# deryrahman/image-caption-emotion-indonesia

Hardware: AMD Instinct MI355X
Metric: images/sec (train step) + NLL loss match, batch=64 ResNet152+FactoredLSTM-512 (higher is better)
Workload: dtype f32 (trunk: operands as 2 f16 pieces each, 3 MFMA products per multiply, f32 accumulate; decoder: large products as 3 bf16 pieces per operand, 6 MFMA products per multiply, the rest f32 MFMA; the persistent LSTM kernel the trunk's split-f16 scheme)

## Files before the change

### image-caption-emotion-indonesia_amd/csrc/fused_block.hip

```cpp
#include <cstdlib>
#include <type_traits>

#include "common.h"
#include "mfma_core.h"
#include "split_f16.h"
#include "kernels.h"

namespace capnet {
namespace {

__host__ __device__ constexpr int fb_kslot(int g, int j) { return 16 * (j >> 2) + 4 * g + (j & 3); }


__global__ __launch_bounds__(256) void fb_pack_kernel(const float* __restrict__ w, unsigned* __restrict__ img, int C, int MID,
                                                      int role, int wide) {
  const int ew = f16x3_weight_shift(img[1]);
  if (blockIdx.x == 0 && threadIdx.x == 0) { img[0] = (unsigned)ew; img[2] = (unsigned)wide; }
  const float ws = ldexpf(1.f, ew);
  const long cells = (long)C * MID / 8 * 2;
  for (long i = (long)blockIdx.x * blockDim.x + threadIdx.x; i < cells; i += (long)gridDim.x * blockDim.x) {
    long r = i;
    const int lane = (int)(r & 63); r >>= 6;
    const int plane = (int)(r & 1); r >>= 1;
    const float* src;
// ... 109 lines not shown
      }
#pragma unroll
      for (int c = 0; c < 4; ++c) {
        const f32x4 a = {x[0][c], x[1][c], x[2][c], x[3][c]}, b = {x[4][c], x[5][c], x[6][c], x[7][c]};
        h4 ha, la, hb, lb;
        split4(a, ha, la);
        split4(b, hb, lb);
        unsigned char* d = lds + (rg * K + 4 * chq + c) * 16;
        *reinterpret_cast<h8*>(d) = cat8(ha, hb);
        *reinterpret_cast<h8*>(d + kPlane) = cat8(la, lb);
      }
    }
  };
  auto mma = [&]() __attribute__((always_inline)) {
#pragma unroll 2
    for (int k = 0; k < NRG / 2; ++k) {
      const unsigned char* base = lds + ((2 * k + lh) * K + li) * 16;
      h8 ah[NBLK], al[NBLK], bh[NBLK], bl[NBLK];
#pragma unroll
      for (int b = 0; b < NBLK; ++b) {
        ah[b] = *reinterpret_cast<const h8*>(base + (b * 64 + wm * 32) * 16);
        al[b] = *reinterpret_cast<const h8*>(base + (b * 64 + wm * 32) * 16 + kPlane);
        bh[b] = *reinterpret_cast<const h8*>(base + (b * 64 + wn * 32) * 16);
        bl[b] = *reinterpret_cast<const h8*>(base + (b * 64 + wn * 32) * 16 + kPlane);
      }
      int p = 0;
#pragma unroll
      for (int bi = 0; bi < NBLK; ++bi)
#pragma unroll
        for (int bj = bi; bj < NBLK; ++bj, ++p) {
          acc[p] = __builtin_amdgcn_mfma_f32_32x32x16_f16(al[bi], bh[bj], acc[p], 0, 0, 0);
          acc[p] = __builtin_amdgcn_mfma_f32_32x32x16_f16(ah[bi], bl[bj], acc[p], 0, 0, 0);
          acc[p] = __builtin_amdgcn_mfma_f32_32x32x16_f16(ah[bi], bh[bj], acc[p], 0, 0, 0);
        }
    }
  };
  fetch(0);
  for (int st = 0; st < nst; ++st) {
    stage(st);
    __syncthreads();
    fetch(st + 1 < nst ? st + 1 : st);
    mma();
    __syncthreads();
  }
  const float osc = ldexpf(1.f, -2 * g.in_exp);
#pragma unroll
  for (int p = 0; p < NPAIR; ++p) {
#pragma unroll
    for (int r = 0; r < 16; ++r) {
      const int m = wm * 32 + (r & 3) + 8 * (r >> 2) + 4 * lh;
      g.gp[(((long)p * 64 + m) * g.slices + slice) * 64 + wn * 32 + li] = acc[p][r] * osc;
    }
  }
  f32x4* cs_sh = reinterpret_cast<f32x4*>(lds);
  cs_sh[tid] = colsum;
  __syncthreads();
  if (tid < NCQ) {
    f32x4 t = cs_sh[tid];
#pragma unroll
    for (int q = 1; q < 256 / NCQ; ++q) t += cs_sh[q * NCQ + tid];
    *reinterpret_cast<f32x4*>(g.cs + (long)slice * K + 4 * tid) = t * ldexpf(1.f, -g.in_exp);
  }
}

__global__ __launch_bounds__(256) void fb_gram_reduce_kernel(const float* __restrict__ gp, const float* __restrict__ cs, float* __restrict__ G,
                                                             float* __restrict__ mu, int K, int slices, int pairs) {
  __shared__ double sh[8][32][4];
  const int it = threadIdx.x & 31, part = threadIdx.x >> 5;
  const int item_wgs = pairs * 32;
  if ((int)blockIdx.x < item_wgs) {
    const int item = blockIdx.x * 32 + it;
    const int n4 = item & 15, m = (item >> 4) & 63, pair = item >> 10;
    const float* p = gp + ((long)(pair * 64 + m) * slices) * 64 + 4 * n4;
    double s[4] = {0.0, 0.0, 0.0, 0.0};
    for (int s0 = part; s0 < slices; s0 += 64) {
      f32x4 v[8];
#pragma unroll
      for (int u = 0; u < 8; ++u) {
        const int sl = s0 + 8 * u;
        v[u] = *reinterpret_cast<const f32x4*>(p + (long)(sl < slices ? sl : part) * 64);
      }
#pragma unroll
      for (int u = 0; u < 8; ++u)
#pragma unroll
        for (int i = 0; i < 4; ++i) s[i] += (s0 + 8 * u < slices) ? (double)v[u][i] : 0.0;
    }
#pragma unroll
    for (int i = 0; i < 4; ++i) sh[part][it][i] = s[i];
    __syncthreads();
    if (part == 0) {
#pragma unroll
      for (int q = 1; q < 8; ++q)
#pragma unroll
        for (int i = 0; i < 4; ++i) s[i] += sh[q][it][i];
      const int nb = K / 64;
      int bi = 0, bj = pair;
      while (bj >= nb - bi) { bj -= nb - bi; ++bi; }
      bj += bi;
      const int r = bi * 64 + m, c = bj * 64 + 4 * n4;
      const f32x4 o = {(float)s[0], (float)s[1], (float)s[2], (float)s[3]};
      *reinterpret_cast<f32x4*>(G + (long)r * K + c) = o;
      if (bi < bj) {
#pragma unroll
        for (int i = 0; i < 4; ++i) G[(long)(c + i) * K + r] = o[i];
      }
    }
  } else {
    const int e = ((int)blockIdx.x - item_wgs) * 32 + it;
    double s = 0.0;
    if (e < K) {
      const float* p = cs + e;
      for (int s0 = part; s0 < slices; s0 += 64) {
        float v[8];
#pragma unroll
        for (int u = 0; u < 8; ++u) {
          const int sl = s0 + 8 * u;
          v[u] = p[(long)(sl < slices ? sl : part) * K];
        }
#pragma unroll
        for (int u = 0; u < 8; ++u) s += (s0 + 8 * u < slices) ? (double)v[u] : 0.0;
      }
    }
    sh[part][it][0] = s;
    __syncthreads();
    if (part == 0 && e < K) {
#pragma unroll
      for (int q = 1; q < 8; ++q) s += sh[q][it][0];
      mu[e] = (float)s;
    }
  }
}

constexpr int kQC = 16;

template <int K>
__global__ __launch_bounds__(K * 4) void fb_quad_kernel(const float* __restrict__ G, const float* __restrict__ mu,
                                                        const float* __restrict__ w , int C, double inv_count,
                                                        double unbias, const float* __restrict__ gamma, const float* __restrict__ beta,
                                                        float* __restrict__ running_mean, float* __restrict__ running_var,
                                                        float momentum, float eps, float* __restrict__ scale, float* __restrict__ shift,
                                                        float* __restrict__ batch_mean, float* __restrict__ batch_var, int* __restrict__ err) {
  constexpr int NW = K / 16, S = K / 4, SB = S < 32 ? S : 32;
  __shared__ float red[2][kQC][NW];
  const int tid = threadIdx.x, lane = tid & 63, nb = tid >> 6, g4 = lane >> 4, ln = lane & 15, c0 = blockIdx.x * kQC;
  const float* wq = w + (long)blockIdx.x * K * kQC;
  f32x4 acc = {0.f, 0.f, 0.f, 0.f};
#pragma unroll
  for (int s0 = 0; s0 < S; s0 += SB) {
    float a[SB], b[SB];
#pragma unroll
    for (int i = 0; i < SB; ++i) {
      const int k = 4 * (s0 + i) + g4;
      a[i] = wq[k * kQC + ln];
      b[i] = G[(long)k * K + 16 * nb + ln];
    }
#pragma unroll
    for (int i = 0; i < SB; ++i) acc = __builtin_amdgcn_mfma_f32_16x16x4f32(a[i], b[i], acc, 0, 0, 0);
  }
  const int col = 16 * nb + ln;
  const f32x4 wv = *reinterpret_cast<const f32x4*>(wq + col * kQC + 4 * g4);
  const float m = mu[col];
#pragma unroll
  for (int r = 0; r < 4; ++r) {
    float q = acc[r] * wv[r], sm = m * wv[r];
#pragma unroll
    for (int o = 1; o < 16; o <<= 1) {
      q += __shfl_xor(q, o);
      sm += __shfl_xor(sm, o);
    }
    if (ln == 0) { red[0][4 * g4 + r][nb] = q; red[1][4 * g4 + r][nb] = sm; }
  }
  __syncthreads();
  if (tid < kQC && c0 + tid < C) {
    const int c = c0 + tid;
    double qq = 0.0, ss = 0.0;
#pragma unroll
    for (int v = 0; v < NW; ++v) { qq += (double)red[0][tid][v]; ss += (double)red[1][tid][v]; }
    if (err && !(qq < __builtin_inf())) atomicOr(err, 8);
    const double mean = ss * inv_count;
    double var = qq * inv_count - mean * mean;
    if (var < 0.0) var = 0.0;
    const float invstd = (float)(1.0 / sqrt(var + (double)eps));
    const float gm = gamma ? gamma[c] : 1.f, bt = beta ? beta[c] : 0.f;
    const float sc = gm * invstd;
    scale[c] = sc;
    shift[c] = bt - (float)mean * sc;
    if (running_mean) {
      running_mean[c] = __builtin_fmaf(momentum, (float)mean, (1.f - momentum) * running_mean[c]);
      running_var[c] = __builtin_fmaf(momentum, (float)(var * unbias), (1.f - momentum) * running_var[c]);
    }
    if (batch_mean) {
      batch_mean[c] = (float)mean;
      batch_var[c] = (float)(var * unbias);
    }
  }
}

struct FArgs {
  const float* y2; const float* s2; const float* t2;
  const unsigned* w3; const unsigned* w1;
  const float* s3; const float* t3;
  const float* res; const float* sd; const float* td;
  float* out; float* y1; float* part_sum; float* part_sq;
  int M, e3, e1;
  int* err;
};

#ifndef CAPNET_FB_DBG
#define CAPNET_FB_DBG 0
#endif

template <int MID, int RS, int NW>
__global__ __launch_bounds__(64 * NW, NW / 4) void fb_fused_kernel(const FArgs g) {
  constexpr int C = 4 * MID, KS = MID / 32, NB = MID / 16, NCH = C / 32;
  constexpr int SLOT = MID * 128;
  constexpr int NDMA = SLOT / 1024 / NW;
  constexpr int L = 2 * RS;
  constexpr int TR = 16 * RS * NW;
  constexpr int NT = 64 * NW;
  static_assert(NDMA >= 1 && 4 * NDMA + 2 * L <= 63, "vmcnt range");
  __shared__ __attribute__((aligned(16))) unsigned char ring[4 * SLOT];
  __shared__ __attribute__((aligned(16))) float par[4][C];
  const int tid = threadIdx.x, lane = tid & 63, wave = tid >> 6, gq = lane >> 4, ln = lane & 15;
  const int wave_u = __builtin_amdgcn_readfirstlane(wave);
  const unsigned ring0 = __builtin_amdgcn_readfirstlane((unsigned)(size_t)(__attribute__((address_space(3))) unsigned char*)ring);
  const int tile0 = (int)blockIdx.x * TR;
  const bool fold_res = g.sd != nullptr;
  const float* const w3img = reinterpret_cast<const float*>(g.w3 + kF16x3HdrWords);
  const float* const w1img = reinterpret_cast<const float*>(g.w1 + kF16x3HdrWords);

  auto dma = [&](const float* img, int cc, int slot) __attribute__((always_inline)) {
    const float* src = img + (long)cc * (SLOT / 4);
#pragma unroll
    for (int q = 0; q < ((CAPNET_FB_DBG == 2 || CAPNET_FB_DBG == 4) ? 0 : NDMA); ++q)
      glds16(src, (wave_u * NDMA + q) * 1024 + lane * 16, ring0 + (unsigned)(slot * SLOT + (wave_u * NDMA + q) * 1024));
  };
  unsigned idoff[RS];
#pragma unroll
  for (int s = 0; s < RS; ++s) {
    const int row = min(tile0 + (wave * RS + s) * 16 + ln, g.M - 1);
    idoff[s] = (unsigned)(((long)row * C + 4 * gq) * 4);
  }
  f32x4 idA[RS][2], idB[RS][2];
  auto fetch_id = [&](int cc, f32x4 (&id)[RS][2]) __attribute__((always_inline)) {
#pragma unroll
    for (int s = 0; s < RS; ++s)
#pragma unroll
      for (int blk = 0; blk < 2; ++blk) gload16(id[s][blk], g.res, idoff[s] + (unsigned)((32 * cc + 16 * blk) * 4));
  };

  dma(w3img, 0, 0);
  dma(w1img, 0, 1);
  fetch_id(0, idA);
  fetch_id(NCH > 1 ? 1 : 0, idB);
  {
    const float x3 = f16x3_out_scale(g.w3[0], g.e3);
    for (int i = tid; i < C; i += NT) {
      par[0][i] = g.s3[i] * x3;
      par[1][i] = g.t3[i];
      par[2][i] = fold_res ? g.sd[i] : 1.f;
      par[3][i] = fold_res ? g.td[i] : 0.f;
    }
  }
  h8 ah[RS][KS], al[RS][KS];
  {
    const float is3 = ldexpf(1.f, g.e3);
#pragma unroll
    for (int s = 0; s < RS; ++s) {
      const int row = min(tile0 + (wave * RS + s) * 16 + ln, g.M - 1);
      const float* p = g.y2 + (long)row * MID + 4 * gq;
#pragma unroll
      for (int ks = 0; ks < KS; ++ks) {
        f32x4 v0 = *reinterpret_cast<const f32x4*>(p + 32 * ks), v1 = *reinterpret_cast<const f32x4*>(p + 32 * ks + 16);
        const f32x4 sa = *reinterpret_cast<const f32x4*>(g.s2 + 32 * ks + 4 * gq), sb = *reinterpret_cast<const f32x4*>(g.s2 + 32 * ks + 16 + 4 * gq);
        const f32x4 ta = *reinterpret_cast<const f32x4*>(g.t2 + 32 * ks + 4 * gq), tb = *reinterpret_cast<const f32x4*>(g.t2 + 32 * ks + 16 + 4 * gq);
#pragma unroll
        for (int e = 0; e < 4; ++e) {
          v0[e] = fmaxf(fmaf(v0[e], sa[e], ta[e]), 0.f) * is3;
          v1[e] = fmaxf(fmaf(v1[e], sb[e], tb[e]), 0.f) * is3;
        }
        h4 h0, l0, h1, l1;
        split4(v0, h0, l0);
        split4(v1, h1, l1);
        ah[s][ks] = cat8(h0, h1);
        al[s][ks] = cat8(l0, l1);
      }
    }
  }
  wait_vmcnt<0>();
  CAPNET_LANDED4(idA[0][0], idA[0][1], idB[0][0], idB[0][1]);
  if constexpr (RS == 2) CAPNET_LANDED4(idA[1][0], idA[1][1], idB[1][0], idB[1][1]);
  __syncthreads();

  f32x4 acc[RS][NB];
#pragma unroll
  for (int s = 0; s < RS; ++s)
#pragma unroll
    for (int nb = 0; nb < NB; ++nb) acc[s][nb] = f32x4{0.f, 0.f, 0.f, 0.f};
  const float is1 = ldexpf(1.f, g.e1);

#ifndef CAPNET_FB_GB8
#define CAPNET_FB_GB8 2
#endif
  constexpr int GB = NW == 8 ? CAPNET_FB_GB8 : 4;
#ifndef CAPNET_FB_FD
#define CAPNET_FB_FD 1
#endif
  constexpr int FD = CAPNET_FB_FD;
  typedef const __attribute__((address_space(3))) unsigned char* lds_bytes;
  const lds_bytes ring3 = (lds_bytes)ring;
  f32x4 d[RS][2];
  auto phase_a = [&](int cc) __attribute__((always_inline)) {
#pragma unroll
    for (int s = 0; s < RS; ++s) { d[s][0] = f32x4{0.f, 0.f, 0.f, 0.f}; d[s][1] = f32x4{0.f, 0.f, 0.f, 0.f}; }
    unsigned wa_off = (unsigned)(((2 * cc) & 3) * SLOT + lane * 16);
    asm volatile("" : "+v"(wa_off));
    const lds_bytes wa = ring3 + wa_off;
    constexpr int GA = KS * 2, NBAT = (GA + GB - 1) / GB;
    h8 f[FD + 1][GB][2];
    auto read_a = [&](int bb) __attribute__((always_inline)) {
#pragma unroll
      for (int q = 0; q < GB; ++q) {
        const int grp = bb * GB + q;
        if (grp < GA && CAPNET_FB_DBG < 3) {
          f[bb % (FD + 1)][q][0] = *(const __attribute__((address_space(3))) h8*)(wa + (grp * 2) * 1024);
          f[bb % (FD + 1)][q][1] = *(const __attribute__((address_space(3))) h8*)(wa + (grp * 2 + 1) * 1024);
        }
      }
    };
#pragma unroll
    for (int bb = 0; bb < FD; ++bb)
      if (bb < NBAT) read_a(bb);
#pragma unroll
    for (int b = 0; b < NBAT; ++b) {
      if (b + FD < NBAT) read_a(b + FD);
      __builtin_amdgcn_sched_barrier(0);
#pragma unroll
      for (int q = 0; q < GB; ++q) {
        const int grp = b * GB + q, ks = grp >> 1, blk = grp & 1;
        if (grp < GA) {
#pragma unroll
          for (int s = 0; s < RS; ++s) {
            if (CAPNET_FB_DBG >= 3) continue;
            if (CAPNET_FB_DBG == 1) { asm volatile("" :: "v"(f[b % (FD + 1)][q][1]), "v"(f[b % (FD + 1)][q][0])); continue; }
            d[s][blk] = __builtin_amdgcn_mfma_f32_16x16x32_f16(f[b % (FD + 1)][q][1], ah[s][ks], d[s][blk], 0, 0, 0);
            d[s][blk] = __builtin_amdgcn_mfma_f32_16x16x32_f16(f[b % (FD + 1)][q][0], al[s][ks], d[s][blk], 0, 0, 0);
            d[s][blk] = __builtin_amdgcn_mfma_f32_16x16x32_f16(f[b % (FD + 1)][q][0], ah[s][ks], d[s][blk], 0, 0, 0);
          }
        }
      }
      __builtin_amdgcn_sched_barrier(0);
    }
  };
  auto phase_b = [&](int cc, f32x4 (&id)[RS][2]) __attribute__((always_inline)) {
    unsigned wb_off = (unsigned)(((2 * cc + 1) & 3) * SLOT + lane * 16);
    asm volatile("" : "+v"(wb_off));
    const lds_bytes wb = ring3 + wb_off;
    constexpr int NBATB = (NB + GB - 1) / GB;
    h8 fb[FD + 1][GB][2];
    auto read_b = [&](int bb) __attribute__((always_inline)) {
#pragma unroll
      for (int q = 0; q < GB; ++q) {
        const int nb = bb * GB + q;
        if (nb < NB && CAPNET_FB_DBG < 3) {
          fb[bb % (FD + 1)][q][0] = *(const __attribute__((address_space(3))) h8*)(wb + (nb * 2) * 1024);
          fb[bb % (FD + 1)][q][1] = *(const __attribute__((address_space(3))) h8*)(wb + (nb * 2 + 1) * 1024);
        }
      }
    };
#pragma unroll
    for (int bb = 0; bb < FD; ++bb)
      if (bb < NBATB) read_b(bb);
    __builtin_amdgcn_sched_barrier(0);
    wait_vmcnt<4 * NDMA + 2 * L>();
    if constexpr (RS == 2) CAPNET_LANDED4(id[0][0], id[0][1], id[1][0], id[1][1]);
    else CAPNET_LANDED2(id[0][0], id[0][1]);
    h8 oh[RS], ol[RS];
#pragma unroll
    for (int s = 0; s < RS; ++s) {
      const int row = min(tile0 + (wave * RS + s) * 16 + ln, g.M - 1);
      h4 hh[2], ll[2];
#pragma unroll
      for (int blk = 0; blk < 2; ++blk) {
        const int ch = 32 * cc + 16 * blk + 4 * gq;
        const f32x4 sv = *reinterpret_cast<const f32x4*>(&par[0][ch]), tv = *reinterpret_cast<const f32x4*>(&par[1][ch]);
        f32x4 r = id[s][blk], o;
        if (fold_res) {
          const f32x4 dv = *reinterpret_cast<const f32x4*>(&par[2][ch]), ev = *reinterpret_cast<const f32x4*>(&par[3][ch]);
#pragma unroll
          for (int e = 0; e < 4; ++e) r[e] = fmaf(r[e], dv[e], ev[e]);
        }
#pragma unroll
        for (int e = 0; e < 4; ++e) o[e] = fmaxf(fmaf(d[s][blk][e], sv[e], tv[e]) + r[e], 0.f);
        *reinterpret_cast<f32x4*>(g.out + (long)row * C + ch) = o;
        split4(o * is1, hh[blk], ll[blk]);
      }
      oh[s] = cat8(hh[0], hh[1]);
      ol[s] = cat8(ll[0], ll[1]);
    }
    fetch_id(cc + 2 < NCH ? cc + 2 : NCH - 1, id);
#pragma unroll
    for (int b = 0; b < NBATB; ++b) {
      if (b + FD < NBATB) read_b(b + FD);
      __builtin_amdgcn_sched_barrier(0);
#pragma unroll
      for (int q = 0; q < GB; ++q) {
        const int nb = b * GB + q;
        if (nb < NB) {
#pragma unroll
          for (int s = 0; s < RS; ++s) {
            if (CAPNET_FB_DBG >= 3) continue;
            if (CAPNET_FB_DBG == 1) { asm volatile("" :: "v"(fb[b % (FD + 1)][q][1]), "v"(fb[b % (FD + 1)][q][0])); continue; }
            acc[s][nb] = __builtin_amdgcn_mfma_f32_16x16x32_f16(ol[s], fb[b % (FD + 1)][q][0], acc[s][nb], 0, 0, 0);
            acc[s][nb] = __builtin_amdgcn_mfma_f32_16x16x32_f16(oh[s], fb[b % (FD + 1)][q][1], acc[s][nb], 0, 0, 0);
            acc[s][nb] = __builtin_amdgcn_mfma_f32_16x16x32_f16(oh[s], fb[b % (FD + 1)][q][0], acc[s][nb], 0, 0, 0);
          }
        }
      }
      __builtin_amdgcn_sched_barrier(0);
    }
  };
  auto head = [&](int k) __attribute__((always_inline)) {
    if (k < 4) wait_vmcnt<0>(); else wait_vmcnt<NDMA + 2 * L>();
    __syncthreads();
    const int p = k + 2 < 2 * NCH ? k + 2 : 2 * NCH - 2 + (k & 1);
    dma((p & 1) ? w1img : w3img, p >> 1, (k + 2) & 3);
  };
  static_assert(NCH % 2 == 0, "chunks come in pairs (two named register sets)");
  auto run = [&](auto lag_c) __attribute__((always_inline)) {
    constexpr int LAG = decltype(lag_c)::value;
    for (int k = 0; k < 2 * NCH; k += 4) {
      const int c0 = k >> 1;
      head(k);
      if constexpr (LAG == 0) phase_a(c0);
      else { if (c0 > 0) phase_b(c0 - 1, idB); }
      head(k + 1);
      if constexpr (LAG == 0) phase_b(c0, idA);
      else phase_a(c0);
      head(k + 2);
      if constexpr (LAG == 0) phase_a(c0 + 1);
      else phase_b(c0, idA);
      head(k + 3);
      if constexpr (LAG == 0) phase_b(c0 + 1, idB);
      else phase_a(c0 + 1);
    }
    if constexpr (NW == 8) {
      head(2 * NCH);
      if constexpr (LAG != 0) phase_b(NCH - 1, idB);
    }
    wait_vmcnt<0>();
    CAPNET_LANDED4(idA[0][0], idA[0][1], idB[0][0], idB[0][1]);
    if constexpr (RS == 2) CAPNET_LANDED4(idA[1][0], idA[1][1], idB[1][0], idB[1][1]);
  };
  if (NW == 4 || wave_u < 4) run(std::integral_constant<int, 0>{});
  else run(std::integral_constant<int, 1>{});
  __syncthreads();

  const float osc = f16x3_out_scale(g.w1[0], g.e1);
  float (*const scratch)[NW][MID] = reinterpret_cast<float (*)[NW][MID]>(ring);
  float bad = 0.f;
#pragma unroll
  for (int nb = 0; nb < NB; ++nb) {
    float cs = 0.f, cq = 0.f;
#pragma unroll
    for (int s = 0; s < RS; ++s)
#pragma unroll
      for (int i = 0; i < 4; ++i) {
        const int row = tile0 + (wave * RS + s) * 16 + 4 * gq + i;
        const float v = acc[s][nb][i] * osc;
        if (row < g.M) {
          g.y1[(long)row * MID + 16 * nb + ln] = v;
          cs += v;
          cq = fmaf(v, v, cq);
        }
      }
    if (g.part_sum) {
      cs += __shfl_xor(cs, 16); cq += __shfl_xor(cq, 16);
      cs += __shfl_xor(cs, 32); cq += __shfl_xor(cq, 32);
      if (gq == 0) { scratch[0][wave][16 * nb + ln] = cs; scratch[1][wave][16 * nb + ln] = cq; }
    } else {
      bad += cq;
    }
  }
  if (!g.part_sum) {
    if (g.err) flag_nonfinite(bad, g.err);
    return;
  }
  __syncthreads();
  for (int c = tid; c < MID; c += NT) {
    float a = 0.f, b = 0.f;
#pragma unroll
    for (int w = 0; w < NW; ++w) { a += scratch[0][w][c]; b += scratch[1][w][c]; }
    g.part_sum[(long)blockIdx.x * MID + c] = a;
    g.part_sq[(long)blockIdx.x * MID + c] = b;
  }
}

template <int MID>
__global__ __launch_bounds__(256, 1) void fb_fused_wide_kernel(const FArgs g) {
  constexpr int C = 4 * MID, KS = MID / 16, NB = MID / 32, NCH = C / 32, NW = 4;
  constexpr int SLOT = MID * 128;
  constexpr int NDMA = SLOT / 1024 / NW;
  constexpr int L = 4;
  constexpr int TR = 32 * NW;
  constexpr int NT = 64 * NW;
  static_assert(NDMA >= 1 && 4 * NDMA + 2 * L <= 63, "vmcnt range");
  __shared__ __attribute__((aligned(16))) unsigned char ring[4 * SLOT];
  __shared__ __attribute__((aligned(16))) float par[4][C];
  const int tid = threadIdx.x, lane = tid & 63, wave = tid >> 6, lh = lane >> 5, li = lane & 31;
  const int wave_u = __builtin_amdgcn_readfirstlane(wave);
  const unsigned ring0 = __builtin_amdgcn_readfirstlane((unsigned)(size_t)(__attribute__((address_space(3))) unsigned char*)ring);
  const int tile0 = (int)blockIdx.x * TR;
  const bool fold_res = g.sd != nullptr;
  const float* const w3img = reinterpret_cast<const float*>(g.w3 + kF16x3HdrWords);
  const float* const w1img = reinterpret_cast<const float*>(g.w1 + kF16x3HdrWords);
  auto dma = [&](const float* img, int cc, int slot) __attribute__((always_inline)) {
    const float* src = img + (long)cc * (SLOT / 4);
#pragma unroll
    for (int q = 0; q < ((CAPNET_FB_DBG == 2 || CAPNET_FB_DBG == 4) ? 0 : NDMA); ++q)
      glds16(src, (wave_u * NDMA + q) * 1024 + lane * 16, ring0 + (unsigned)(slot * SLOT + (wave_u * NDMA + q) * 1024));
  };
  const int myrow = min(tile0 + wave * 32 + li, g.M - 1);
  const unsigned idoff = (unsigned)(((long)myrow * C + 4 * lh) * 4);
  f32x4 idA[4], idB[4];
  auto fetch_id = [&](int cc, f32x4 (&id)[4]) __attribute__((always_inline)) {
#pragma unroll
    for (int q = 0; q < 4; ++q) gload16(id[q], g.res, idoff + (unsigned)((32 * cc + 8 * q) * 4));
  };
  dma(w3img, 0, 0);
  dma(w1img, 0, 1);
  fetch_id(0, idA);
  fetch_id(NCH > 1 ? 1 : 0, idB);
  {
    const float x3 = f16x3_out_scale(g.w3[0], g.e3);
    for (int i = tid; i < C; i += NT) {
      par[0][i] = g.s3[i] * x3;
      par[1][i] = g.t3[i];
      par[2][i] = fold_res ? g.sd[i] : 1.f;
      par[3][i] = fold_res ? g.td[i] : 0.f;
    }
  }
  h8 ah[KS], al[KS];
  {
    const float is3 = ldexpf(1.f, g.e3);
    const float* p = g.y2 + (long)myrow * MID + 8 * lh;
#pragma unroll
    for (int ks = 0; ks < KS; ++ks) {
      f32x4 v0 = *reinterpret_cast<const f32x4*>(p + 16 * ks), v1 = *reinterpret_cast<const f32x4*>(p + 16 * ks + 4);
      const f32x4 sa = *reinterpret_cast<const f32x4*>(g.s2 + 16 * ks + 8 * lh), sb = *reinterpret_cast<const f32x4*>(g.s2 + 16 * ks + 8 * lh + 4);
      const f32x4 ta = *reinterpret_cast<const f32x4*>(g.t2 + 16 * ks + 8 * lh), tb = *reinterpret_cast<const f32x4*>(g.t2 + 16 * ks + 8 * lh + 4);
#pragma unroll
      for (int e = 0; e < 4; ++e) {
        v0[e] = fmaxf(fmaf(v0[e], sa[e], ta[e]), 0.f) * is3;
        v1[e] = fmaxf(fmaf(v1[e], sb[e], tb[e]), 0.f) * is3;
      }
      h4 h0, l0, h1, l1;
      split4(v0, h0, l0);
      split4(v1, h1, l1);
      ah[ks] = cat8(h0, h1);
      al[ks] = cat8(l0, l1);
    }
  }
  wait_vmcnt<0>();
  CAPNET_LANDED4(idA[0], idA[1], idA[2], idA[3]);
  CAPNET_LANDED4(idB[0], idB[1], idB[2], idB[3]);
  __syncthreads();

  f32x16 acc[NB];
#pragma unroll
  for (int nb = 0; nb < NB; ++nb)
#pragma unroll
    for (int r = 0; r < 16; ++r) acc[nb][r] = 0.f;
  const float is1 = ldexpf(1.f, g.e1);
  typedef const __attribute__((address_space(3))) unsigned char* lds_bytes;
  typedef const __attribute__((address_space(3))) h8* lds_h8;
  const lds_bytes ring3 = (lds_bytes)ring;
  constexpr int GB = 4;
  f32x16 d;
  auto phase_a = [&](int cc) __attribute__((always_inline)) {
#pragma unroll
    for (int r = 0; r < 16; ++r) d[r] = 0.f;
    unsigned wa_off = (unsigned)(((2 * cc) & 3) * SLOT + lane * 16);
    asm volatile("" : "+v"(wa_off));
    const lds_bytes wa = ring3 + wa_off;
    constexpr int NBAT = (KS + GB - 1) / GB;
    h8 f[2][GB][2];
#pragma unroll
    for (int q = 0; q < GB; ++q)
      if (q < KS) { f[0][q][0] = *(lds_h8)(wa + (q * 2) * 1024); f[0][q][1] = *(lds_h8)(wa + (q * 2 + 1) * 1024); }
#pragma unroll
    for (int b = 0; b < NBAT; ++b) {
      if (b + 1 < NBAT) {
#pragma unroll
        for (int q = 0; q < GB; ++q) {
          const int ks = (b + 1) * GB + q;
          if (ks < KS) { f[(b + 1) & 1][q][0] = *(lds_h8)(wa + (ks * 2) * 1024); f[(b + 1) & 1][q][1] = *(lds_h8)(wa + (ks * 2 + 1) * 1024); }
        }
      }
      __builtin_amdgcn_sched_barrier(0);
#pragma unroll
      for (int q = 0; q < GB; ++q) {
        const int ks = b * GB + q;
        if (ks < KS) {
          d = __builtin_amdgcn_mfma_f32_32x32x16_f16(f[b & 1][q][1], ah[ks], d, 0, 0, 0);
          d = __builtin_amdgcn_mfma_f32_32x32x16_f16(f[b & 1][q][0], al[ks], d, 0, 0, 0);
          d = __builtin_amdgcn_mfma_f32_32x32x16_f16(f[b & 1][q][0], ah[ks], d, 0, 0, 0);
        }
      }
      __builtin_amdgcn_sched_barrier(0);
    }
  };
  auto phase_b = [&](int cc, f32x4 (&id)[4]) __attribute__((always_inline)) {
    unsigned wb_off = (unsigned)(((2 * cc + 1) & 3) * SLOT + lane * 16);
    asm volatile("" : "+v"(wb_off));
    const lds_bytes wb = ring3 + wb_off;
    constexpr int NG = NB * 2, NBATB = (NG + GB - 1) / GB;
    h8 fb[2][GB][2];
#pragma unroll
    for (int q = 0; q < GB; ++q)
      if (q < NG) { fb[0][q][0] = *(lds_h8)(wb + (q * 2) * 1024); fb[0][q][1] = *(lds_h8)(wb + (q * 2 + 1) * 1024); }
    __builtin_amdgcn_sched_barrier(0);
    wait_vmcnt<4 * NDMA + 2 * L>();
    CAPNET_LANDED4(id[0], id[1], id[2], id[3]);
    h4 hh[4], ll[4];
#pragma unroll
    for (int q = 0; q < 4; ++q) {
      const int ch = 32 * cc + 8 * q + 4 * lh;
      const f32x4 sv = *reinterpret_cast<const f32x4*>(&par[0][ch]), tv = *reinterpret_cast<const f32x4*>(&par[1][ch]);
      f32x4 r = id[q], o;
      if (fold_res) {
        const f32x4 dv = *reinterpret_cast<const f32x4*>(&par[2][ch]), ev = *reinterpret_cast<const f32x4*>(&par[3][ch]);
#pragma unroll
        for (int e = 0; e < 4; ++e) r[e] = fmaf(r[e], dv[e], ev[e]);
      }
#pragma unroll
      for (int e = 0; e < 4; ++e) o[e] = fmaxf(fmaf(d[4 * q + e], sv[e], tv[e]) + r[e], 0.f);
      *reinterpret_cast<f32x4*>(g.out + (long)myrow * C + ch) = o;
      split4(o * is1, hh[q], ll[q]);
    }
    const h8 oh[2] = {cat8(hh[0], hh[1]), cat8(hh[2], hh[3])}, ol[2] = {cat8(ll[0], ll[1]), cat8(ll[2], ll[3])};
    fetch_id(cc + 2 < NCH ? cc + 2 : NCH - 1, id);
#pragma unroll
    for (int b = 0; b < NBATB; ++b) {
      if (b + 1 < NBATB) {
#pragma unroll
        for (int q = 0; q < GB; ++q) {
          const int grp = (b + 1) * GB + q;
          if (grp < NG) { fb[(b + 1) & 1][q][0] = *(lds_h8)(wb + (grp * 2) * 1024); fb[(b + 1) & 1][q][1] = *(lds_h8)(wb + (grp * 2 + 1) * 1024); }
        }
      }
      __builtin_amdgcn_sched_barrier(0);
#pragma unroll
      for (int q = 0; q < GB; ++q) {
        const int grp = b * GB + q, nb = grp >> 1, st = grp & 1;
        if (grp < NG) {
          acc[nb] = __builtin_amdgcn_mfma_f32_32x32x16_f16(ol[st], fb[b & 1][q][0], acc[nb], 0, 0, 0);
          acc[nb] = __builtin_amdgcn_mfma_f32_32x32x16_f16(oh[st], fb[b & 1][q][1], acc[nb], 0, 0, 0);
          acc[nb] = __builtin_amdgcn_mfma_f32_32x32x16_f16(oh[st], fb[b & 1][q][0], acc[nb], 0, 0, 0);
        }
      }
      __builtin_amdgcn_sched_barrier(0);
    }
  };
  auto head = [&](int k) __attribute__((always_inline)) {
    if (k < 4) wait_vmcnt<0>(); else wait_vmcnt<NDMA + 2 * L>();
    __syncthreads();
    const int p = k + 2 < 2 * NCH ? k + 2 : 2 * NCH - 2 + (k & 1);
    dma((p & 1) ? w1img : w3img, p >> 1, (k + 2) & 3);
  };
  static_assert(NCH % 2 == 0, "chunks come in pairs (two named register sets)");
  for (int k = 0; k < 2 * NCH; k += 4) {
    const int c0 = k >> 1;
    head(k);
    phase_a(c0);
    head(k + 1);
    phase_b(c0, idA);
    head(k + 2);
    phase_a(c0 + 1);
    head(k + 3);
    phase_b(c0 + 1, idB);
  }
  wait_vmcnt<0>();
  CAPNET_LANDED4(idA[0], idA[1], idA[2], idA[3]);
  CAPNET_LANDED4(idB[0], idB[1], idB[2], idB[3]);
  __syncthreads();

  const float osc = f16x3_out_scale(g.w1[0], g.e1);
  float (*const scratch)[NW][MID] = reinterpret_cast<float (*)[NW][MID]>(ring);
  float bad = 0.f;
#pragma unroll
  for (int nb = 0; nb < NB; ++nb) {
    float cs = 0.f, cq = 0.f;
#pragma unroll
    for (int r = 0; r < 16; ++r) {
      const int row = tile0 + wave * 32 + (r & 3) + 8 * (r >> 2) + 4 * lh;
      const float v = acc[nb][r] * osc;
      if (row < g.M) {
        g.y1[(long)row * MID + 32 * nb + li] = v;
        cs += v;
        cq = fmaf(v, v, cq);
      }
    }
    if (g.part_sum) {
      cs += __shfl_xor(cs, 32); cq += __shfl_xor(cq, 32);
      if (lh == 0) { scratch[0][wave][32 * nb + li] = cs; scratch[1][wave][32 * nb + li] = cq; }
    } else {
      bad += cq;
    }
  }
  if (!g.part_sum) {
    if (g.err) flag_nonfinite(bad, g.err);
    return;
  }
  __syncthreads();
  for (int c = tid; c < MID; c += NT) {
    float a = 0.f, b = 0.f;
#pragma unroll
    for (int w = 0; w < NW; ++w) { a += scratch[0][w][c]; b += scratch[1][w][c]; }
    g.part_sum[(long)blockIdx.x * MID + c] = a;
    g.part_sq[(long)blockIdx.x * MID + c] = b;
  }
}

}

bool fused_block_shape_ok(long M, int MID) {
  return (MID == 64 || MID == 128 || MID == 256) && M > 0 && M < (1l << 24) && M * 4 * MID * 4 < (1l << 32);
}

size_t fused_block_weight_words(int C, int MID, int role) {
  return (size_t)kF16x3HdrWords + (size_t)C * MID * (role == 0 ? 2 : 1);
}

static bool fb_wide(int MID) {
  const char* e = getenv("CAPNET_FB_WIDE");
  if (e && (e[0] == '0' || e[0] == '1')) return e[0] == '1';
  (void)MID;
  return false;
}

int fused_block_pack(const float* w, unsigned* img, int C, int MID, int role, hipStream_t stream) {
  CAPNET_REQUIRE(w && img && aligned16(img) && C == 4 * MID && (MID == 64 || MID == 128 || MID == 256) && (role == 0 || role == 1),
                 "fused_block_pack: bad argument (C=%d MID=%d role=%d)", C, MID, role);
  const long n = (long)C * MID;
  const int rh = f16x3_pack_header(w, img, n, stream);
  if (rh) return rh;
  hipLaunchKernelGGL(fb_pack_kernel, dim3((int)(cdiv(n / 4, 256) > 2048 ? 2048 : cdiv(n / 4, 256))), dim3(256), 0, stream, w, img, C, MID, role, fb_wide(MID) ? 1 : 0);
  CAPNET_LAUNCH_CHECK();
  return kOk;
}

int fused_block_gram_slices(long M, int K) { return cdiv(M, fb_gram_rows(K)); }
int fused_block_gram_pairs(int K) { const int nb = K / 64; return nb * (nb + 1) / 2; }
size_t fused_block_stats_floats(long M, int K) {
  const size_t s = fused_block_gram_slices(M, K), p = fused_block_gram_pairs(K);
  return s * p * 4096 + ((s * K + 3) / 4 * 4) + ((size_t)K * K + K) + 8;
}

int fused_block_stats(const float* y2, const float* s2, const float* t2, const unsigned* w3img, long M, int MID, int in_exp,
                      const float* gamma, const float* beta, float* running_mean, float* running_var, float momentum, float eps,
                      float* scale, float* shift, float* batch_mean, float* batch_var, float* work, int* err, hipStream_t stream) {
  CAPNET_REQUIRE(y2 && s2 && t2 && w3img && scale && shift && work && aligned16(work) && aligned16(y2) && fused_block_shape_ok(M, MID) &&
                     in_exp > -64 && in_exp < 64, "fused_block_stats: bad argument");
  const int K = MID, C = 4 * MID;
  GArgs a;
  a.y2 = y2; a.s2 = s2; a.t2 = t2; a.M = (int)M; a.K = K; a.in_exp = in_exp;
  a.slices = fused_block_gram_slices(M, K); a.pairs = fused_block_gram_pairs(K); a.slice_rows = fb_gram_rows(K);
  a.gp = work;
  a.cs = work + (size_t)a.slices * a.pairs * 4096;
  float* G = a.cs + ((size_t)a.slices * K + 3) / 4 * 4;
  float* mu = G + (size_t)K * K;
  if (K == 256) hipLaunchKernelGGL(fb_gram_kernel<256>, dim3(a.slices), dim3(256), 0, stream, a);
  else if (K == 128) hipLaunchKernelGGL(fb_gram_kernel<128>, dim3(a.slices), dim3(256), 0, stream, a);
  else hipLaunchKernelGGL(fb_gram_kernel<64>, dim3(a.slices), dim3(256), 0, stream, a);
  hipLaunchKernelGGL(fb_gram_reduce_kernel, dim3(a.pairs * 32 + K / 32), dim3(256), 0, stream, a.gp, a.cs, G, mu, K, a.slices, a.pairs);
  const double inv = 1.0 / (double)M, unbias = M > 1 ? (double)M / (double)(M - 1) : 1.0;
  const float* wcopy = reinterpret_cast<const float*>(w3img + kF16x3HdrWords + (size_t)C * MID);
  if (K == 256)
    hipLaunchKernelGGL(fb_quad_kernel<256>, dim3(cdiv(C, kQC)), dim3(K * 4), 0, stream, G, mu, wcopy, C, inv, unbias, gamma, beta,
                       running_mean, running_var, momentum, eps, scale, shift, batch_mean, batch_var, err);
  else if (K == 128)
    hipLaunchKernelGGL(fb_quad_kernel<128>, dim3(cdiv(C, kQC)), dim3(K * 4), 0, stream, G, mu, wcopy, C, inv, unbias, gamma, beta,
                       running_mean, running_var, momentum, eps, scale, shift, batch_mean, batch_var, err);
  else
    hipLaunchKernelGGL(fb_quad_kernel<64>, dim3(cdiv(C, kQC)), dim3(K * 4), 0, stream, G, mu, wcopy, C, inv, unbias, gamma, beta,
                       running_mean, running_var, momentum, eps, scale, shift, batch_mean, batch_var, err);
  CAPNET_LAUNCH_CHECK();
  return kOk;
}

static void fb_shape(int MID, int* rs, int* nw) {
  (void)MID;
  const char* e = getenv("CAPNET_FB_RS");
  const char* w = getenv("CAPNET_FB_NW");
  *nw = (w && w[0] == '4') ? 4 : 8;
  *rs = (e && (e[0] == '1' || e[0] == '2')) ? e[0] - '0' : (*nw == 8 ? 1 : 2);
  if (*nw == 8) *rs = 1;
}
int fused_block_tiles(long M, int MID) {
  if (fb_wide(MID)) return cdiv(M, 128);
  int rs, nw;
  fb_shape(MID, &rs, &nw);
  return cdiv(M, 16 * rs * nw);
}

int fused_block_forward(const float* y2, const float* s2, const float* t2, const unsigned* w3img, const float* s3, const float* t3,
                        const float* res, const float* sd, const float* td, float* out, const unsigned* w1img, float* y1,
                        float* part_sum, float* part_sq, long M, int MID, int e3, int e1, int* err, hipStream_t stream) {
  CAPNET_REQUIRE(y2 && s2 && t2 && w3img && s3 && t3 && res && out && w1img && y1 && fused_block_shape_ok(M, MID),
                 "fused_block_forward: bad argument");
  CAPNET_REQUIRE(aligned16(y2) && aligned16(s2) && aligned16(t2) && aligned16(w3img) && aligned16(w1img) && aligned16(res) &&
                     aligned16(out) && (sd == nullptr) == (td == nullptr) && (part_sum == nullptr) == (part_sq == nullptr) &&
                     e3 > -64 && e3 < 64 && e1 > -64 && e1 < 64, "fused_block_forward: alignment / pairs / exponents");
  FArgs a;
  a.y2 = y2; a.s2 = s2; a.t2 = t2; a.w3 = w3img; a.w1 = w1img; a.s3 = s3; a.t3 = t3; a.res = res; a.sd = sd; a.td = td;
  a.out = out; a.y1 = y1; a.part_sum = part_sum; a.part_sq = part_sq; a.M = (int)M; a.e3 = e3; a.e1 = e1; a.err = err;
  const dim3 grid(fused_block_tiles(M, MID));
  int rs, nw;
  fb_shape(MID, &rs, &nw);
  if (fb_wide(MID)) {
    const dim3 block(256);
    if (MID == 256) CAPNET_LAUNCH_TIMED((fb_fused_wide_kernel<256>), grid, block, stream, a);
    else if (MID == 128) CAPNET_LAUNCH_TIMED((fb_fused_wide_kernel<128>), grid, block, stream, a);
    else CAPNET_LAUNCH_TIMED((fb_fused_wide_kernel<64>), grid, block, stream, a);
    CAPNET_LAUNCH_CHECK();
    return kOk;
  }
  const dim3 block(64 * nw);
  if (nw == 8) {
    if (MID == 256) CAPNET_LAUNCH_TIMED((fb_fused_kernel<256, 1, 8>), grid, block, stream, a);
    else if (MID == 128) CAPNET_LAUNCH_TIMED((fb_fused_kernel<128, 1, 8>), grid, block, stream, a);
    else CAPNET_LAUNCH_TIMED((fb_fused_kernel<64, 1, 8>), grid, block, stream, a);
  } else if (rs == 2) {
    if (MID == 256) CAPNET_LAUNCH_TIMED((fb_fused_kernel<256, 2, 4>), grid, block, stream, a);
    else if (MID == 128) CAPNET_LAUNCH_TIMED((fb_fused_kernel<128, 2, 4>), grid, block, stream, a);
    else CAPNET_LAUNCH_TIMED((fb_fused_kernel<64, 2, 4>), grid, block, stream, a);
  } else {
    if (MID == 256) CAPNET_LAUNCH_TIMED((fb_fused_kernel<256, 1, 4>), grid, block, stream, a);
    else if (MID == 128) CAPNET_LAUNCH_TIMED((fb_fused_kernel<128, 1, 4>), grid, block, stream, a);
    else CAPNET_LAUNCH_TIMED((fb_fused_kernel<64, 1, 4>), grid, block, stream, a);
  }
  CAPNET_LAUNCH_CHECK();
  return kOk;
}

}
```

### image-caption-emotion-indonesia_amd/csrc/mfma_core.h

```cpp
#pragma once
#include <hip/hip_runtime.h>

#include "step_core.h"

namespace capnet {

typedef float f32x16 __attribute__((ext_vector_type(16)));

constexpr int kGemmThreads = 256;

template <int BM_, int BN_, int BK_>
struct TileCfg {
  static constexpr int BM = BM_, BN = BN_, BK = BK_;
  static constexpr int LDA = BM + 4;
  static constexpr int LDB = BN + 4;
  static constexpr int A_ELEMS = BK * LDA;
  static constexpr int B_ELEMS = BK * LDB;
  static constexpr int STAGE_ELEMS = A_ELEMS + B_ELEMS;
  static constexpr int LDS_BYTES = 2 * STAGE_ELEMS * 4;
  static constexpr int MT = BM / 64;
  static constexpr int NT = BN / 64;
  static_assert(BM % 64 == 0 && BN % 64 == 0, "wave grid is 2x2 of 32-multiples");
  static_assert(BK % 8 == 0, "BK");
};


__device__ __forceinline__ float4 mask4(float4 v, int n) {
  v.x = n > 0 ? v.x : 0.f;
  v.y = n > 1 ? v.y : 0.f;
  v.z = n > 2 ? v.z : 0.f;
  v.w = n > 3 ? v.w : 0.f;
  return v;
}

__device__ __forceinline__ float4 load4_scalar(const float* __restrict__ p, int n) {
  float4 v = make_float4(0.f, 0.f, 0.f, 0.f);
  if (n > 0) v.x = p[0];
  if (n > 1) v.y = p[1];
  if (n > 2) v.z = p[2];
  if (n > 3) v.w = p[3];
  return v;
}

template <int BR, int BK, int LD, bool VEC>
struct LoaderKContig {
  static constexpr int TPR = BK / 4;
  static constexpr int RPP = kGemmThreads / TPR;
  static constexpr int PASSES = BR / RPP;
  static_assert(BR % RPP == 0, "tile rows vs threads");
  const float* p;
  long ld;
  int R, K, r0;
  float4 v[PASSES];
  int nv[PASSES];
  __device__ __forceinline__ void init(const float* p_, long ld_, int R_, int K_, int r0_) {
    p = p_; ld = ld_; R = R_; K = K_; r0 = r0_;
  }
  __device__ __forceinline__ void load(int k0) {
    const int kc = threadIdx.x % TPR, rl = threadIdx.x / TPR;
    const int k = k0 + 4 * kc;
    int kn = K - k;
    kn = kn < 0 ? 0 : (kn > 4 ? 4 : kn);
    const int kk = kn > 0 ? k : 0;
#pragma unroll
    for (int ps = 0; ps < PASSES; ++ps) {
      const int r = r0 + rl + ps * RPP;
      const bool rv = r < R;
      const int rr = rv ? r : R - 1;
      nv[ps] = rv ? kn : 0;
      if (VEC) v[ps] = *reinterpret_cast<const float4*>(p + (long)rr * ld + kk);
      else v[ps] = load4_scalar(p + (long)rr * ld + kk, nv[ps]);
    }
  }
  __device__ __forceinline__ void store(float* lds) const {
    const int kc = threadIdx.x % TPR, rl = threadIdx.x / TPR;
#pragma unroll
    for (int ps = 0; ps < PASSES; ++ps) {
      const float4 t = mask4(v[ps], nv[ps]);
      float* d = lds + (4 * kc) * LD + rl + ps * RPP;
      d[0 * LD] = t.x;
      d[1 * LD] = t.y;
      d[2 * LD] = t.z;
      d[3 * LD] = t.w;
    }
  }
};

template <int BR, int BK, int LD, bool VEC>
struct LoaderRContig {
  static constexpr int TPK = BR / 4;
  static constexpr int KPP = kGemmThreads / TPK;
  static constexpr int PASSES = (BK + KPP - 1) / KPP;
  static_assert(kGemmThreads % TPK == 0, "tile rows vs threads");
  const float* p;
  long ld;
  int R, K, r0;
  float4 v[PASSES];
  int nv[PASSES];
  __device__ __forceinline__ void init(const float* p_, long ld_, int R_, int K_, int r0_) {
    p = p_; ld = ld_; R = R_; K = K_; r0 = r0_;
  }
  __device__ __forceinline__ void load(int k0) {
    const int rc = threadIdx.x % TPK, kl = threadIdx.x / TPK;
    const int r = r0 + 4 * rc;
    int rn = R - r;
    rn = rn < 0 ? 0 : (rn > 4 ? 4 : rn);
    const int rr = rn > 0 ? r : 0;
#pragma unroll
    for (int ps = 0; ps < PASSES; ++ps) {
      const int kk = kl + ps * KPP;
      const int k = k0 + kk;
      const bool kv = k < K && kk < BK;
      const int kc = k < K ? k : K - 1;
      nv[ps] = kv ? rn : 0;
      if (VEC) v[ps] = *reinterpret_cast<const float4*>(p + (long)kc * ld + rr);
      else v[ps] = load4_scalar(p + (long)kc * ld + rr, nv[ps]);
    }
  }
  __device__ __forceinline__ void store(float* lds) const {
    const int rc = threadIdx.x % TPK, kl = threadIdx.x / TPK;
#pragma unroll
    for (int ps = 0; ps < PASSES; ++ps) {
      const int kk = kl + ps * KPP;
      if (kk < BK) *reinterpret_cast<float4*>(lds + kk * LD + 4 * rc) = mask4(v[ps], nv[ps]);
    }
  }
};

template <class T, class AL, class BL>
__device__ __forceinline__ void gemm_block_mainloop(AL& al, BL& bl, int K, float* lds,
                                                    f32x16 (&acc)[T::MT][T::NT]) {
  const int lane = threadIdx.x & 63, wave = threadIdx.x >> 6;
  const int wm = wave >> 1, wn = wave & 1;
  const int li = lane & 31, lh = lane >> 5;
#pragma unroll
  for (int mt = 0; mt < T::MT; ++mt)
#pragma unroll
    for (int nt = 0; nt < T::NT; ++nt)
#pragma unroll
      for (int r = 0; r < 16; ++r) acc[mt][nt][r] = 0.f;

  const int nk = (K + T::BK - 1) / T::BK;
  al.load(0);
  bl.load(0);
  al.store(lds);
  bl.store(lds + T::A_ELEMS);
  __syncthreads();
  for (int kt = 0; kt < nk; ++kt) {
    float* cur = lds + (kt & 1) * T::STAGE_ELEMS;
    float* nxt = lds + ((kt + 1) & 1) * T::STAGE_ELEMS;
    const bool more = (kt + 1) < nk;
    if (more) {
      al.load((kt + 1) * T::BK);
      bl.load((kt + 1) * T::BK);
    }
    const float* As = cur + lh * T::LDA + wm * (T::BM / 2) + li;
    const float* Bs = cur + T::A_ELEMS + lh * T::LDB + wn * (T::BN / 2) + li;
    float a0[T::MT], b0[T::NT], a1[T::MT], b1[T::NT];
#pragma unroll
    for (int mt = 0; mt < T::MT; ++mt) a0[mt] = As[mt * 32];
#pragma unroll
    for (int nt = 0; nt < T::NT; ++nt) b0[nt] = Bs[nt * 32];
#pragma unroll
    for (int j = 0; j < T::BK / 2; j += 2) {
#pragma unroll
      for (int mt = 0; mt < T::MT; ++mt) a1[mt] = As[(2 * j + 2) * T::LDA + mt * 32];
#pragma unroll
      for (int nt = 0; nt < T::NT; ++nt) b1[nt] = Bs[(2 * j + 2) * T::LDB + nt * 32];
      __builtin_amdgcn_sched_barrier(0);
#pragma unroll
      for (int mt = 0; mt < T::MT; ++mt)
#pragma unroll
        for (int nt = 0; nt < T::NT; ++nt)
          acc[mt][nt] = __builtin_amdgcn_mfma_f32_32x32x2f32(a0[mt], b0[nt], acc[mt][nt], 0, 0, 0);
      __builtin_amdgcn_sched_barrier(0);
      if (j + 2 < T::BK / 2) {
#pragma unroll
        for (int mt = 0; mt < T::MT; ++mt) a0[mt] = As[(2 * j + 4) * T::LDA + mt * 32];
#pragma unroll
        for (int nt = 0; nt < T::NT; ++nt) b0[nt] = Bs[(2 * j + 4) * T::LDB + nt * 32];
      }
      __builtin_amdgcn_sched_barrier(0);
#pragma unroll
      for (int mt = 0; mt < T::MT; ++mt)
#pragma unroll
        for (int nt = 0; nt < T::NT; ++nt)
          acc[mt][nt] = __builtin_amdgcn_mfma_f32_32x32x2f32(a1[mt], b1[nt], acc[mt][nt], 0, 0, 0);
    }
    if (more) {
      al.store(nxt);
      bl.store(nxt + T::A_ELEMS);
    }
    __syncthreads();
  }
}

__device__ __forceinline__ int xcd_remap(int id, int nwg) {
  const int q = nwg >> 3, r = nwg & 7;
  const int xcd = id & 7, within = id >> 3;
  const int base = (xcd < r) ? xcd * (q + 1) : r * (q + 1) + (xcd - r) * q;
  return base + within;
}

template <class T>
__device__ __forceinline__ void block_col_stats(const f32x16 (&acc)[T::MT][T::NT], float* lds,
                                                float* __restrict__ out_sum,
                                                float* __restrict__ out_sq, int n0, int N) {
  const int lane = threadIdx.x & 63, wave = threadIdx.x >> 6;
  const int wm = wave >> 1, wn = wave & 1;
  const int li = lane & 31, lh = lane >> 5;
  float* s_sum = lds;
  float* s_sq = lds + 2 * T::BN;
#pragma unroll
  for (int nt = 0; nt < T::NT; ++nt) {
    float s = 0.f, q = 0.f;
#pragma unroll
    for (int mt = 0; mt < T::MT; ++mt)
#pragma unroll
      for (int r = 0; r < 16; ++r) {
        const float x = acc[mt][nt][r];
        s += x;
        q = fmaf(x, x, q);
      }
    s += __shfl_xor(s, 32);
    q += __shfl_xor(q, 32);
    if (lh == 0) {
      const int c = wn * (T::BN / 2) + nt * 32 + li;
      s_sum[wm * T::BN + c] = s;
      s_sq[wm * T::BN + c] = q;
    }
  }
  __syncthreads();
  for (int c = threadIdx.x; c < T::BN; c += kGemmThreads) {
    if (n0 + c < N) {
      out_sum[n0 + c] = s_sum[c] + s_sum[T::BN + c];
      out_sq[n0 + c] = s_sq[c] + s_sq[T::BN + c];
    }
  }
}

__device__ __forceinline__ void flag_nonfinite(float t, int* err) {
  if (!(t < __builtin_inff())) atomicOr(err, 8);
}


static inline void magic_div(unsigned d, unsigned* mul, unsigned* sh) {
  unsigned l = 0;
  while ((1u << l) < d) ++l;
  const unsigned k = 24 + l;
  const unsigned long long m = ((1ull << k) + d - 1) / d;
  *mul = (unsigned)m;
  *sh = k;
}
__device__ __forceinline__ unsigned fast_div(unsigned n, unsigned mul, unsigned sh) {
  return (unsigned)(((unsigned long long)n * mul) >> sh);
}

__device__ __forceinline__ void glds16(const float* sbase, int voff_bytes, unsigned lds_byte_addr) {
  unsigned keep;
  asm volatile(
      "s_mov_b32 %0, m0\n\t"
      "s_mov_b32 m0, %2\n\t"
      "s_nop 2\n\t"
      "global_load_lds_dwordx4 %1, %3\n\t"
      "s_mov_b32 m0, %0"
      : "=&s"(keep)
      : "v"(voff_bytes), "s"(lds_byte_addr), "s"(sbase)
      : "memory");
}

__device__ __forceinline__ void gload16(f32x4& dst, const float* sbase, unsigned voff_bytes) {
  asm volatile("s_nop 4\n\tglobal_load_dwordx4 %0, %1, %2" : "=&v"(dst) : "v"(voff_bytes), "s"(sbase) : "memory");
}
__device__ __forceinline__ void gstore32(float* base, unsigned off_bytes, float v) {
  float* p = reinterpret_cast<float*>(reinterpret_cast<char*>(base) + off_bytes);
  asm volatile("global_store_dword %0, %1, off" ::"v"(p), "v"(v) : "memory");
}
#define CAPNET_LANDED_IN1(a) asm volatile("; capnet.landed %0" ::"v"(a) : "memory")
#define CAPNET_LANDED_IN4(a, b, c, d) asm volatile("; capnet.landed %0 %1 %2 %3" ::"v"(a), "v"(b), "v"(c), "v"(d) : "memory")
#define CAPNET_LANDED1(a) asm volatile("; capnet.landed %0" : "+v"(a)::"memory")
#define CAPNET_LANDED2(a, b) asm volatile("; capnet.landed %0 %1" : "+v"(a), "+v"(b)::"memory")
#define CAPNET_LANDED4(a, b, c, d) \
  asm volatile("; capnet.landed %0 %1 %2 %3" : "+v"(a), "+v"(b), "+v"(c), "+v"(d)::"memory")

}
```

Baseline: 9046.

## Enable two row-slabs per wave in 8-wave fused bottleneck kernel for MID 64/128

The 8-wave fused bottleneck kernel now defaults to two 16-row slabs per wave (RS=2) for MID 64 and 128, so one block covers 256 rows and each loaded weight fragment is reused across more rows. The partial-sum epilogue is split into two 128-row partial rows, so the BN statistics layout stays unchanged and fused_block_tiles still reports 128-row tiles. Output stores in that variant use an inline-asm global_store_dwordx4 with a scalar base, and the MFMA batch size drops to 1 for MID>=128 to limit register pressure. The larger per-wave state risks lower occupancy or register spills, and the grid now has fewer blocks.

```diff
diff --git a/image-caption-emotion-indonesia_amd/csrc/fused_block.hip b/image-caption-emotion-indonesia_amd/csrc/fused_block.hip
--- a/image-caption-emotion-indonesia_amd/csrc/fused_block.hip
+++ b/image-caption-emotion-indonesia_amd/csrc/fused_block.hip
@@ -435,7 +435,7 @@
 #ifndef CAPNET_FB_GB8
 #define CAPNET_FB_GB8 2
 #endif
-  constexpr int GB = NW == 8 ? CAPNET_FB_GB8 : 4;
+  constexpr int GB = NW != 8 ? 4 : (RS == 2 && MID >= 128) ? 1 : CAPNET_FB_GB8;
 #ifndef CAPNET_FB_FD
 #define CAPNET_FB_FD 1
 #endif
@@ -525,7 +525,8 @@
         }
 #pragma unroll
         for (int e = 0; e < 4; ++e) o[e] = fmaxf(fmaf(d[s][blk][e], sv[e], tv[e]) + r[e], 0.f);
-        *reinterpret_cast<f32x4*>(g.out + (long)row * C + ch) = o;
+        if constexpr (RS == 2 && NW == 8) gstore16(g.out, idoff[s] + (unsigned)((32 * cc + 16 * blk) * 4), o);
+        else *reinterpret_cast<f32x4*>(g.out + (long)row * C + ch) = o;
         split4(o * is1, hh[blk], ll[blk]);
       }
       oh[s] = cat8(hh[0], hh[1]);
@@ -589,30 +590,42 @@
   else run(std::integral_constant<int, 1>{});
   __syncthreads();
 
+  constexpr int PR = (RS == 2 && NW == 8) ? 2 : 1;
+  constexpr int SP = PR == 2 ? RS : 1;
+  constexpr int NS = NW * SP;
+  static_assert(2 * NS * MID * 4 <= 4 * SLOT, "the ring holds the epilogue's sums");
+  int tid_e = tid;
+  asm volatile("" : "+v"(tid_e));
+  const int wave_e = tid_e >> 6, gq_e = (tid_e >> 4) & 3, ln_e = tid_e & 15;
   const float osc = f16x3_out_scale(g.w1[0], g.e1);
-  float (*const scratch)[NW][MID] = reinterpret_cast<float (*)[NW][MID]>(ring);
+  float (*const scratch)[NS][MID] = reinterpret_cast<float (*)[NS][MID]>(ring);
   float bad = 0.f;
 #pragma unroll
   for (int nb = 0; nb < NB; ++nb) {
-    float cs = 0.f, cq = 0.f;
+    float cs[SP], cq[SP];
+#pragma unroll
+    for (int u = 0; u < SP; ++u) { cs[u] = 0.f; cq[u] = 0.f; }
 #pragma unroll
     for (int s = 0; s < RS; ++s)
 #pragma unroll
       for (int i = 0; i < 4; ++i) {
-        const int row = tile0 + (wave * RS + s) * 16 + 4 * gq + i;
+        const int row = tile0 + (wave_e * RS + s) * 16 + 4 * gq_e + i;
         const float v = acc[s][nb][i] * osc;
         if (row < g.M) {
-          g.y1[(long)row * MID + 16 * nb + ln] = v;
-          cs += v;
-          cq = fmaf(v, v, cq);
-        }
-      }
-    if (g.part_sum) {
-      cs += __shfl_xor(cs, 16); cq += __shfl_xor(cq, 16);
-      cs += __shfl_xor(cs, 32); cq += __shfl_xor(cq, 32);
-      if (gq == 0) { scratch[0][wave][16 * nb + ln] = cs; scratch[1][wave][16 * nb + ln] = cq; }
-    } else {
-      bad += cq;
+          g.y1[(long)row * MID + 16 * nb + ln_e] = v;
+          cs[SP == 1 ? 0 : s] += v;
+          cq[SP == 1 ? 0 : s] = fmaf(v, v, cq[SP == 1 ? 0 : s]);
+        }
+      }
+#pragma unroll
+    for (int u = 0; u < SP; ++u) {
+      if (g.part_sum) {
+        cs[u] += __shfl_xor(cs[u], 16); cq[u] += __shfl_xor(cq[u], 16);
+        cs[u] += __shfl_xor(cs[u], 32); cq[u] += __shfl_xor(cq[u], 32);
+        if (gq_e == 0) { scratch[0][wave_e * SP + u][16 * nb + ln_e] = cs[u]; scratch[1][wave_e * SP + u][16 * nb + ln_e] = cq[u]; }
+      } else {
+        bad += cq[u];
+      }
     }
   }
   if (!g.part_sum) {
@@ -620,12 +633,15 @@
     return;
   }
   __syncthreads();
-  for (int c = tid; c < MID; c += NT) {
+  const int prows = PR == 2 ? (g.M + 127) / 128 : (int)gridDim.x;
+  for (int c = tid_e; c < MID * PR; c += NT) {
+    const int h = c / MID, col = c - h * MID, prow = (int)blockIdx.x * PR + h;
+    if (prow >= prows) continue;
     float a = 0.f, b = 0.f;
 #pragma unroll
-    for (int w = 0; w < NW; ++w) { a += scratch[0][w][c]; b += scratch[1][w][c]; }
-    g.part_sum[(long)blockIdx.x * MID + c] = a;
-    g.part_sq[(long)blockIdx.x * MID + c] = b;
+    for (int w = 0; w < NS / PR; ++w) { a += scratch[0][h * (NS / PR) + w][col]; b += scratch[1][h * (NS / PR) + w][col]; }
+    g.part_sum[(long)prow * MID + col] = a;
+    g.part_sq[(long)prow * MID + col] = b;
   }
 }
 
@@ -922,19 +938,30 @@
   return kOk;
 }
 
+static constexpr bool fb_rs8_has2(int MID) { return MID == 64 || MID == 128; }
+static constexpr int fb_rs8_default(int MID) { return (MID == 64 || MID == 128) ? 2 : 1; }
 static void fb_shape(int MID, int* rs, int* nw) {
-  (void)MID;
   const char* e = getenv("CAPNET_FB_RS");
   const char* w = getenv("CAPNET_FB_NW");
+  const int ers = (e && (e[0] == '1' || e[0] == '2')) ? e[0] - '0' : 0;
   *nw = (w && w[0] == '4') ? 4 : 8;
-  *rs = (e && (e[0] == '1' || e[0] == '2')) ? e[0] - '0' : (*nw == 8 ? 1 : 2);
-  if (*nw == 8) *rs = 1;
+  if (*nw == 4) { *rs = ers ? ers : 2; return; }
+  *rs = ers ? ers : fb_rs8_default(MID);
+  const char* only = getenv("CAPNET_FB_RS2_MID");
+  if (only && only[0] && atoi(only) != MID) *rs = 1;
+  if (!fb_rs8_has2(MID)) *rs = 1;
+}
+static int fb_grid(long M, int MID) {
+  if (fb_wide(MID)) return cdiv(M, 128);
+  int rs, nw;
+  fb_shape(MID, &rs, &nw);
+  return cdiv(M, 16 * rs * nw);
 }
 int fused_block_tiles(long M, int MID) {
   if (fb_wide(MID)) return cdiv(M, 128);
   int rs, nw;
   fb_shape(MID, &rs, &nw);
-  return cdiv(M, 16 * rs * nw);
+  return cdiv(M, nw == 8 ? 128 : 16 * rs * nw);
 }
 
 int fused_block_forward(const float* y2, const float* s2, const float* t2, const unsigned* w3img, const float* s3, const float* t3,
@@ -948,7 +975,7 @@
   FArgs a;
   a.y2 = y2; a.s2 = s2; a.t2 = t2; a.w3 = w3img; a.w1 = w1img; a.s3 = s3; a.t3 = t3; a.res = res; a.sd = sd; a.td = td;
   a.out = out; a.y1 = y1; a.part_sum = part_sum; a.part_sq = part_sq; a.M = (int)M; a.e3 = e3; a.e1 = e1; a.err = err;
-  const dim3 grid(fused_block_tiles(M, MID));
+  const dim3 grid(fb_grid(M, MID));
   int rs, nw;
   fb_shape(MID, &rs, &nw);
   if (fb_wide(MID)) {
@@ -960,7 +987,10 @@
     return kOk;
   }
   const dim3 block(64 * nw);
-  if (nw == 8) {
+  if (nw == 8 && rs == 2) {
+    if (MID == 128) CAPNET_LAUNCH_TIMED((fb_fused_kernel<128, 2, 8>), grid, block, stream, a);
+    else CAPNET_LAUNCH_TIMED((fb_fused_kernel<64, 2, 8>), grid, block, stream, a);
+  } else if (nw == 8) {
     if (MID == 256) CAPNET_LAUNCH_TIMED((fb_fused_kernel<256, 1, 8>), grid, block, stream, a);
     else if (MID == 128) CAPNET_LAUNCH_TIMED((fb_fused_kernel<128, 1, 8>), grid, block, stream, a);
     else CAPNET_LAUNCH_TIMED((fb_fused_kernel<64, 1, 8>), grid, block, stream, a);
diff --git a/image-caption-emotion-indonesia_amd/csrc/mfma_core.h b/image-caption-emotion-indonesia_amd/csrc/mfma_core.h
--- a/image-caption-emotion-indonesia_amd/csrc/mfma_core.h
+++ b/image-caption-emotion-indonesia_amd/csrc/mfma_core.h
@@ -276,6 +276,9 @@
   float* p = reinterpret_cast<float*>(reinterpret_cast<char*>(base) + off_bytes);
   asm volatile("global_store_dword %0, %1, off" ::"v"(p), "v"(v) : "memory");
 }
+__device__ __forceinline__ void gstore16(float* sbase, unsigned voff_bytes, const f32x4& v) {
+  asm volatile("s_nop 4\n\tglobal_store_dwordx4 %0, %1, %2" ::"v"(voff_bytes), "v"(v), "s"(sbase) : "memory");
+}
 #define CAPNET_LANDED_IN1(a) asm volatile("; capnet.landed %0" ::"v"(a) : "memory")
 #define CAPNET_LANDED_IN4(a, b, c, d) asm volatile("; capnet.landed %0 %1 %2 %3" ::"v"(a), "v"(b), "v"(c), "v"(d) : "memory")
 #define CAPNET_LANDED1(a) asm volatile("; capnet.landed %0" : "+v"(a)::"memory")
```

After: 9222, median of 6. 1.9% higher.
